# pkuyzy/ESC-GNN

Hardware: AMD Instinct MI355X
Metric: graphs/sec + edges-aggregated/sec, NestedGIN_eff h=3 bs=128 @1/2/4/8 GPU (higher is better)
Workload: dtype f32; 1 GPU; count_cycle-shaped random regular graphs (n in 10/15/20/30), target=triangles, NestedGIN_eff h=3 layers=4 hidden=256, bs=128 per GPU (configs[1]); global_batch=128, parallelism=dp1 graph-sharded, rccl_ranks=1, ranks=1

## Files before the change

esc-gnn_amd/csrc/common.h:

```cpp
#pragma once
#include <hip/hip_runtime.h>
#include <hip/hip_ext.h>
#include <stdint.h>
#include <stdio.h>
#include <stdarg.h>

#include "../../include/escgnn_hip.h"

namespace esc {

constexpr int WAVE = 64;

#ifndef ESC_NODE_PRIO
#define ESC_NODE_PRIO 2
#endif
#define ESC_PRIO() __builtin_amdgcn_s_setprio(ESC_NODE_PRIO)

void set_error(const char* fmt, ...);

#define ESC_REQUIRE(cond, ...)                    \
  do {                                            \
    if (!(cond)) {                                \
      esc::set_error(__VA_ARGS__);                \
      return ESC_EINVAL;                          \
// ... 5 lines not shown
    hipError_t err__ = hipGetLastError();                                   \
    if (err__ != hipSuccess) {                                              \
      esc::set_error("%s: launch failed: %s", name, hipGetErrorString(err__)); \
      return ESC_ELAUNCH;                                                   \
    }                                                                       \
  } while (0)

inline bool aligned16(const void* p) { return (reinterpret_cast<uintptr_t>(p) & 15) == 0; }
inline int64_t cdiv(int64_t a, int64_t b) { return (a + b - 1) / b; }

bool prof_slot(int kind, hipEvent_t* start, hipEvent_t* stop);
unsigned long long* prof_span_next(int kind);
#define ESC_SPAN_WGS 2048
#define ESC_SPAN_WAVES 8192
#define ESC_SPAN_STRIDE (ESC_SPAN_WGS + ESC_SPAN_WAVES)
bool trace_launch();

void arm_launch_event(hipEvent_t ev);
hipEvent_t take_launch_event();

template <typename... KArgs, typename... Args>
inline void launch(int kind, void (*kernel)(KArgs...), dim3 grid, dim3 block, size_t lds, hipStream_t s,
                   Args... args) {
  hipEvent_t a = nullptr, b = nullptr;
  hipEvent_t done = take_launch_event();
  if (done != nullptr) {
    hipStreamCaptureStatus cap = hipStreamCaptureStatusNone;
    if (hipStreamIsCapturing(s, &cap) != hipSuccess || cap != hipStreamCaptureStatusNone) { arm_launch_event(done); done = nullptr; }
  }
  if (prof_slot(kind, &a, &b)) {
    hipExtLaunchKernelGGL(kernel, grid, block, (unsigned)lds, s, a, b, 0, static_cast<KArgs>(args)...);
    if (done != nullptr) (void)hipEventRecord(done, s);
  } else if (done != nullptr) {
    hipExtLaunchKernelGGL(kernel, grid, block, (unsigned)lds, s, nullptr, done, 0, static_cast<KArgs>(args)...);
  } else {
    hipLaunchKernelGGL(kernel, grid, block, (unsigned)lds, s, static_cast<KArgs>(args)...);
  }
  if (trace_launch()) {
    const char* name = hipKernelNameRefByPtr(reinterpret_cast<const void*>(kernel), s);
    fprintf(stderr, "[esc] %s grid (%u,%u,%u) block %u lds %zu stream %p ...", name ? name : "?", grid.x, grid.y, grid.z, block.x, lds, (void*)s);
    fflush(stderr);
    const hipError_t e = hipStreamSynchronize(s);
    fprintf(stderr, " %s\n", e == hipSuccess ? "done" : hipGetErrorString(e));
  }
}

struct BnCounters {
  int n = 0;
  int64_t* p[ESC_MAX_BN_COUNTERS] = {};
};
int bag_bwd_classify_counted(const int32_t* c_row, int64_t Z, int64_t H, int64_t rows, float* partials, const BnCounters& cnt,
                             void* stream);

__device__ __forceinline__ int lane_id() { return threadIdx.x & 63; }

__device__ __forceinline__ int uniform(int v) { return __builtin_amdgcn_readfirstlane(v); }

__device__ __forceinline__ float wave_sum(float v) {
#pragma unroll
  for (int o = 32; o > 0; o >>= 1) v += __shfl_xor(v, o, 64);
  return v;
}
__device__ __forceinline__ double wave_sum(double v) {
#pragma unroll
  for (int o = 32; o > 0; o >>= 1) v += __shfl_xor(v, o, 64);
  return v;
}

unsigned* tickets(int n);
int gemm_lds_floor();
void set_gemm_lds_floor(int bytes);
int edge_lds_floor();
int node_lds_floor();
void set_node_lds_floor(int bytes);
void set_edge_lds_floor(int bytes);
int norm_rowblock_cap();
void set_norm_rowblock_cap(int v);
bool bn_bwd_one_launch();
void set_bn_bwd_one_launch(int on);
bool bn_bwd_fold();
void set_bn_bwd_fold(int on);
bool last_block_finalize();
void set_last_block_finalize(int on);
void set_linear_knob(int knob, int value);

__device__ __forceinline__ void store_agent(float2* p, float2 v) {
  const unsigned long long bits = ((unsigned long long)__float_as_uint(v.y) << 32) | __float_as_uint(v.x);
  __hip_atomic_store(reinterpret_cast<unsigned long long*>(p), bits, __ATOMIC_RELAXED, __HIP_MEMORY_SCOPE_AGENT);
}

__device__ __forceinline__ bool grid_last_block(unsigned* counter, unsigned nblocks) {
  __shared__ unsigned s_ticket;
  __builtin_amdgcn_s_waitcnt(0x0F70);
  __syncthreads();
  if (threadIdx.x == 0) s_ticket = __hip_atomic_fetch_add(counter, 1u, __ATOMIC_RELAXED, __HIP_MEMORY_SCOPE_AGENT);
  __syncthreads();
  const bool last = s_ticket == nblocks - 1;
  if (last) {
    __builtin_amdgcn_fence(__ATOMIC_ACQUIRE, "agent");
    if (threadIdx.x == 0) *counter = 0;
  }
  return last;
}

__device__ __forceinline__ void chan_merge(double& n, double& mu, double& m2, double nb, double mub, double m2b) {
  if (nb == 0.0) return;
  const double tot = n + nb;
  const double delta = mub - mu;
  mu += delta * nb / tot;
  m2 += m2b + delta * delta * n * nb / tot;
  n = tot;
}


struct BnFoldDev {
  const float2* partials;
  int P, block_rows, M, C;
  float eps, momentum;
  const float* gamma; const float* beta;
  float* mean; float* invstd; float* scale; float* shift; float* running_mean; float* running_var;
};
__device__ __forceinline__ void bn_fold_column(const BnFoldDev& f, int col, bool writer, float& sc, float& sh) {
  const int full = f.M / f.block_rows;
  double n = 0.0, mu = 0.0, m2 = 0.0;
  if (full > 0) {
    const double pivot = (double)f.partials[col].x;
    double S1 = 0.0, S2 = 0.0, SM = 0.0;
    constexpr int CH = 40;
    for (int p0 = 0; p0 < full; p0 += CH) {
      float2 v[CH];
#pragma unroll
      for (int u = 0; u < CH; ++u) v[u] = f.partials[(size_t)min(p0 + u, full - 1) * f.C + col];
#pragma unroll
      for (int u = 0; u < CH; ++u) {
        if (p0 + u < full) { const double d = (double)v[u].x - pivot; S1 += d; S2 += d * d; SM += (double)v[u].y; }
      }
    }
    n = (double)f.block_rows * full;
    mu = pivot + S1 / full;
    m2 = SM + (double)f.block_rows * (S2 - S1 * S1 / full);
    if (m2 < 0.0) m2 = 0.0;
  }
  if (f.M > f.block_rows * full) {
    const float2 v = f.partials[(size_t)full * f.C + col];
    chan_merge(n, mu, m2, (double)(f.M - f.block_rows * full), (double)v.x, (double)v.y);
  }
  const float is = (float)(1.0 / sqrt(m2 / (double)f.M + (double)f.eps));
  sc = (f.gamma ? f.gamma[col] : 1.f) * is;
  sh = (f.beta ? f.beta[col] : 0.f) - (float)mu * sc;
  if (writer) {
    f.mean[col] = (float)mu;
    f.invstd[col] = is;
    if (f.scale) { f.scale[col] = sc; f.shift[col] = sh; }
    if (f.running_mean) f.running_mean[col] = (1.f - f.momentum) * f.running_mean[col] + f.momentum * (float)mu;
    if (f.running_var) f.running_var[col] = (1.f - f.momentum) * f.running_var[col] + f.momentum * (float)(m2 / (double)(f.M - 1));
  }
}

struct BnbDev {
  const float* x; int ldx;
  const float* mean; const float* invstd; const float* scale; const float* shift;
  const float2* coef;
  int relu;
};
struct BnStatDev {
  float2* partial;
// ... 20 lines not shown
```

esc-gnn_amd/csrc/linear_mfma.hip:

```cpp
#include "common.h"
#include <cstdlib>
#include "linear_plan.h"
#include "gemm_tile.h"
#include "gemm_dma.h"
#include "linear_small.h"
#include "linear_narrow.h"

namespace esc {

using plan::Flags;
using plan::Op;
using plan::Plan;

static plan::PlanKnobs g_plan;
void set_linear_knob(int knob, int value) {
  if (knob == 11) g_plan.use_dma = value;
  else g_plan.knob[knob] = value;
}
static const plan::PlanKnobs& knobs() {
  static const bool env_read = [] {
    if (getenv("ESC_BIG_MIN_WGS")) g_plan.big_min_wgs = atoll(getenv("ESC_BIG_MIN_WGS"));
    if (getenv("ESC_TILE160")) g_plan.tile160 = atoi(getenv("ESC_TILE160"));
    if (getenv("ESC_TILE160_MIN_WGS")) g_plan.tile160_min_wgs = atoll(getenv("ESC_TILE160_MIN_WGS"));
    return true;
// ... 69 lines not shown
static void dma_fill_dx(dma::GArgs& g, const float* dY, int64_t ld_dy, const float* W, int64_t ld_w, int64_t M, int64_t N,
                        int64_t K, float* dX, int64_t ld_dx, int accumulate) {
  g.A = dY; g.lda = (int)ld_dy; g.B = W; g.ldb = (int)ld_w; g.C = dX; g.ldc = (int)ld_dx;
  g.M = (int)M; g.N = (int)K; g.R = (int)N; g.red_per_split = (int)N; g.accumulate = accumulate;
}
static void dma_fill_dw(dma::GArgs& g, const float* dY, int64_t ld_dy, const float* X, int64_t ld_x, const float* in_scale,
                        const float* in_shift, int64_t M, int64_t N, int64_t K, float* slabs, const Plan& p) {
  g.A = dY; g.lda = (int)ld_dy; g.B = X; g.ldb = (int)ld_x; g.C = slabs; g.ldc = (int)K;
  g.pro_scale = in_scale; g.pro_shift = in_shift; g.db_part = slabs + (size_t)p.splits * N * K;
  g.M = (int)N; g.N = (int)K; g.R = (int)M; g.red_per_split = p.per_split; g.accumulate = 0;
}

enum NarrowForm { NARROW_PLAIN, NARROW_FOLD, NARROW_L1 };
static void launch_narrow_fwd(NarrowForm form, const float* X, int64_t ld_x, const float* W, int64_t ld_w, const float* bias,
                              const float* in_scale, const float* in_shift, int64_t M, int64_t N, int64_t K, float* Y, int64_t ld_y,
                              const BnFoldDev& fold, const NarrowL1& l1, hipStream_t s) {
  const unsigned blocks = (unsigned)(cdiv(M, 16) < 2048 ? cdiv(M, 16) : 2048);
#define ESC_NARROW_FWD(...) \
  esc::launch(ESC_K_LINEAR, linear_narrow_fwd<__VA_ARGS__>, dim3(blocks), dim3(256), 0, s, X, ld_x, W, ld_w, bias, in_scale, in_shift, (int)M, (int)N, (int)K, Y, ld_y, fold, l1)
  if (form == NARROW_L1) ESC_NARROW_FWD(1, true, false, true);
  else if (form == NARROW_FOLD) { if (N == 1) ESC_NARROW_FWD(1, true, true); else ESC_NARROW_FWD(4, true, true); }
  else if (N == 1) { if (in_scale) ESC_NARROW_FWD(1, true); else ESC_NARROW_FWD(1, false); }
  else { if (in_scale) ESC_NARROW_FWD(4, true); else ESC_NARROW_FWD(4, false); }
#undef ESC_NARROW_FWD
}

static hipError_t launch_dma_fwd(const Plan& p, const dma::GArgs& g, hipStream_t s) {
  const bool pro = g.pro_scale != nullptr;
#define ESC_DMA_FWD(PRO, ...) dma::launch_gemm<__VA_ARGS__, false, false, PRO, true, false>(g, 0, s)
#define ESC_DMA_FWD_FROM(PRO, ...) dma::launch_gemm<__VA_ARGS__, false, false, PRO, true, false, true>(g, 0, s)
  const bool big = p.family == plan::F_DMA128;
  if (g.c_init != nullptr) {
    if (big) return pro ? ESC_DMA_FWD_FROM(1, ESC_T128) : ESC_DMA_FWD_FROM(0, ESC_T128);
    return pro ? ESC_DMA_FWD_FROM(1, ESC_T64) : ESC_DMA_FWD_FROM(0, ESC_T64);
  }
  if (g.fold.partials != nullptr) return big ? ESC_DMA_FWD(3, ESC_T128) : ESC_DMA_FWD(3, ESC_T64);
  switch (p.family) {
    case plan::F_DMA64X32:
      return pro ? dma::launch_gemm<ESC_T64X32, false, false, 1, false, false>(g, 0, s)
                 : dma::launch_gemm<ESC_T64X32, false, false, 0, false, false>(g, 0, s);
    case plan::F_DMA160: return pro ? ESC_DMA_FWD(1, ESC_T160) : ESC_DMA_FWD(0, ESC_T160);
    case plan::F_DMA128: return pro ? ESC_DMA_FWD(1, ESC_T128) : ESC_DMA_FWD(0, ESC_T128);
    case plan::F_DMA128X64: return ESC_DMA_FWD(0, ESC_T128X64);
    default: return pro ? ESC_DMA_FWD(1, ESC_T64) : ESC_DMA_FWD(0, ESC_T64);
  }
#undef ESC_DMA_FWD
#undef ESC_DMA_FWD_FROM
}
static dma::GArgs dma_fwd_args(const float* X, int64_t ld_x, const float* W, int64_t ld_w, const float* bias, const float* in_scale,
                               const float* in_shift, int64_t M, int64_t N, int64_t K, float* Y, int64_t ld_y, float* col_stats) {
  dma::GArgs g{};
  g.A = X; g.lda = (int)ld_x; g.B = W; g.ldb = (int)ld_w; g.C = Y; g.ldc = (int)ld_y; g.bias = bias;
  g.pro_scale = in_scale; g.pro_shift = in_shift; g.col_stats = reinterpret_cast<float2*>(col_stats);
  g.M = (int)M; g.N = (int)N; g.R = (int)K; g.red_per_split = (int)K; g.accumulate = 0;
  return g;
}

static int launch_smalln_dx(const float* dY, int64_t ld_dy, const float* W, int64_t ld_w, int64_t M, int64_t N, int64_t K, float* dX,
                            int64_t ld_dx, int accumulate, const BnbDev& bd, int act, const char* what, hipStream_t s) {
  const size_t lds = (size_t)(32 + small::SMALL_MAX) * (N + 4) * sizeof(float);
  static size_t raised[3] = {64 * 1024, 64 * 1024, 64 * 1024};
  hipError_t e = hipSuccess;
  if (act == 0) e = dma::raise_lds(small::smalln_dx<small::SMALL_MAX>, lds, raised[0]);
  if (act != 0) e = dma::raise_lds(small::smalln_dx<small::SMALL_MAX, 1>, lds, raised[1]);
  if (e == hipSuccess && act == 2) e = dma::raise_lds(small::smalln_dx<small::SMALL_MAX, 2>, lds, raised[2]);
  if (dma_check(e, what) != hipSuccess) return ESC_ELAUNCH;
  auto kern = act == 0 ? small::smalln_dx<small::SMALL_MAX> : (act == 2 ? small::smalln_dx<small::SMALL_MAX, 2> : small::smalln_dx<small::SMALL_MAX, 1>);
  esc::launch(ESC_K_LINEAR, kern, dim3((unsigned)cdiv(M, 32)), dim3(256), lds, s, dY, ld_dy, W, ld_w, (int)M, (int)N, (int)K, dX, ld_dx, accumulate, bd);
  return ESC_OK;
}

static void launch_wgrad_small(const float* dY, int64_t ld_dy, const float* X, int64_t ld_x, const float* in_scale, const float* in_shift,
                               int64_t M, int64_t N, int64_t K, float* slabs, const Plan& p, const BnbDev& bd, int act, hipStream_t s) {
  float* db_part = slabs + (size_t)p.splits * N * K;
  const bool small_k = K <= small::SMALL_MAX;
  const dim3 grid((unsigned)p.splits, (unsigned)cdiv(small_k ? N : K, 256));
#define ESC_WGRAD_SMALL(...) \
  esc::launch(ESC_K_LINEAR, small::wgrad_small<small::SMALL_MAX, __VA_ARGS__>, grid, dim3(256), 0, s, dY, ld_dy, X, ld_x, in_scale, in_shift, (int)M, (int)N, (int)K, slabs, db_part, bd)
  if (act == 2)      { if (in_scale) ESC_WGRAD_SMALL(true, true, 2); else ESC_WGRAD_SMALL(true, false, 2); }
  else if (act == 1) { if (in_scale) ESC_WGRAD_SMALL(true, true, 1); else ESC_WGRAD_SMALL(true, false, 1); }
  else if (small_k)  { if (in_scale) ESC_WGRAD_SMALL(true, true); else ESC_WGRAD_SMALL(true, false); }
  else               { if (in_scale) ESC_WGRAD_SMALL(false, true); else ESC_WGRAD_SMALL(false, false); }
#undef ESC_WGRAD_SMALL
}

static int reduce_slabs(const Plan& p, const float* slabs, int64_t N, int64_t K, float* dW, int64_t ld_dw, float* db, esc_reduce_job* defer,
                        void* stream) {
  esc_reduce_job now;
  esc_reduce_job* j = defer ? defer : &now;
  j->slabs = slabs; j->n = N * K; j->splits = p.splits; j->cols = K; j->dw = dW; j->ld_dw = ld_dw;
  j->db_part = slabs + (size_t)p.splits * N * K; j->rows = N; j->db = db;
  return defer ? ESC_OK : esc_slab_reduce_jobs(j, 1, stream);
}

}

using namespace esc;

extern "C" {

int esc_debug_gemm_occupancy(int tile_id) {
  int n = -1;
#define ESC_OCC(I)                                                                                                              \
  {                                                                                                                             \
    constexpr plan::Tile t = plan::R01_TILE[I];                                                                                 \
    auto kern = gemm_tile_kernel<t.bm, t.bn, t.wm, t.wn, t.bk, true, true, false, false>;                                       \
    const size_t lds = 2 * (KContigTile<t.bm, t.bk>::FLOATS + KContigTile<t.bn, t.bk>::FLOATS) * sizeof(float);                 \
    if (lds > 64 * 1024) (void)hipFuncSetAttribute((const void*)kern, hipFuncAttributeMaxDynamicSharedMemorySize, (int)lds);    \
    (void)hipOccupancyMaxActiveBlocksPerMultiprocessor(&n, kern, 256, lds);                                                     \
  }
  switch (tile_id) {
    case 0: ESC_OCC(0) break;
    case 2: ESC_OCC(2) break;
    case 3: ESC_OCC(3) break;
    case 4: ESC_OCC(4) break;
    default: ESC_OCC(1) break;
  }
#undef ESC_OCC
  return n;
}

static int linear_fwd_impl(const float* X, int64_t ld_x, const float* W, int64_t ld_w, const float* bias,
                           const float* in_scale, const float* in_shift, int64_t M, int64_t N, int64_t K,
                           float* Y, int64_t ld_y, float* col_stats, const esc_bn_fuse* bn, void* stream) {
  ESC_REQUIRE(X && W && Y, "esc_linear_fwd: null pointer");
  ESC_REQUIRE(M >= 0 && N > 0 && K > 0 && ld_x >= K && ld_w >= K && ld_y >= N, "esc_linear_fwd: bad sizes M=%ld N=%ld K=%ld", (long)M, (long)N, (long)K);
  ESC_REQUIRE((in_scale == nullptr) == (in_shift == nullptr), "esc_linear_fwd: in_scale/in_shift must come together");
  ESC_REQUIRE(col_stats == nullptr || N > 32, "esc_linear_fwd: col_stats needs N > 32");
  ESC_REQUIRE(M < (1LL << 31) && N < (1LL << 31) && K < (1LL << 31), "esc_linear_fwd: dimension too large");
  ESC_REQUIRE(bn == nullptr || (col_stats && bn->mean && bn->invstd && M > 1), "esc_linear_bn_fwd: needs col_stats, mean, invstd and M > 1");
  ESC_REQUIRE(bn == nullptr || ((bn->scale == nullptr) == (bn->shift == nullptr)), "esc_linear_bn_fwd: scale/shift must come together");
  if (M == 0) return ESC_OK;
  hipStream_t s = (hipStream_t)stream;
  Flags f = pro_flags(in_scale, in_shift);
  f.col_stats = col_stats != nullptr; f.bn = bn != nullptr; f.last_block_finalize = last_block_finalize();
  const Plan p = plan::plan_fwd(knobs(), Op{X, ld_x}, Op{W, ld_w}, M, N, K, f);
  switch (p.family) {
    case plan::F_NARROW:
      launch_narrow_fwd(NARROW_PLAIN, X, ld_x, W, ld_w, bias, in_scale, in_shift, M, N, K, Y, ld_y, BnFoldDev{}, NarrowL1{}, s);
      ESC_CHECK_LAUNCH("esc_linear_fwd.narrow");
      break;
    case plan::F_SMALLK:
      esc::launch(ESC_K_LINEAR, small::smallk_fwd<small::SMALL_MAX>, dim3((unsigned)cdiv(M, small::ROWS_FWD), (unsigned)cdiv(N, 256)),
                  dim3(256), 0, s, X, ld_x, W, ld_w, bias, (int)M, (int)N, (int)K, Y, ld_y, reinterpret_cast<float2*>(col_stats));
      ESC_CHECK_LAUNCH("esc_linear_fwd.smallk");
      break;
    case plan::F_DMA64X32: case plan::F_DMA64: case plan::F_DMA128: case plan::F_DMA128X64: case plan::F_DMA160:
      if (dma_check(launch_dma_fwd(p, dma_fwd_args(X, ld_x, W, ld_w, bias, in_scale, in_shift, M, N, K, Y, ld_y, col_stats), s), "esc_linear_fwd") != hipSuccess)
        return ESC_ELAUNCH;
      break;
    default: {
      GemmArgs g{};
      g.A = X; g.lda = ld_x; g.B = W; g.ldb = ld_w; g.C = Y; g.ldc = ld_y; g.bias = bias;
      g.pro_scale = in_scale; g.pro_shift = in_shift; g.db_part = nullptr;
      g.col_stats = p.family == plan::F_R01_ROWSTATS ? nullptr : reinterpret_cast<float2*>(col_stats);
      g.rowsC = (int)M; g.colsC = (int)N; g.red = (int)K; g.red_per_split = (int)K; g.accumulate = 0;
      g.a_vec = plan::vec_ok(Op{X, ld_x}) && f.pro_aligned;
      g.b_vec = plan::vec_ok(Op{W, ld_w}); g.c_slab = 0;
      if (p.family == plan::F_R01_BN) {
        g.fin.tickets = tickets((int)cdiv(N, p.bn));
        ESC_REQUIRE(g.fin.tickets != nullptr, "esc_linear_bn_fwd: no ticket counters");
        g.fin.row_tiles = (int)cdiv(M, p.bm);
        g.fin.eps = bn->eps; g.fin.momentum = bn->momentum; g.fin.mean = bn->mean; g.fin.invstd = bn->invstd;
        g.fin.running_mean = bn->running_mean; g.fin.running_var = bn->running_var; g.fin.gamma = bn->gamma;
        g.fin.beta = bn->beta; g.fin.scale = bn->scale; g.fin.shift = bn->shift;
      }
// ... 221 lines not shown
      dma_fill_dw(a.dw, dY, ld_dy, X, ld_x, in_scale, in_shift, M, N, K, slabs, p);
      hipError_t e;
      if (p.family == plan::F_DMA160_DUAL)      e = in_scale ? dma::launch_dual<ESC_T160, true>(a, 0, s) : dma::launch_dual<ESC_T160, false>(a, 0, s);
      else if (p.family == plan::F_DMA128_DUAL) e = in_scale ? dma::launch_dual<ESC_T128, true>(a, 0, s) : dma::launch_dual<ESC_T128, false>(a, 0, s);
      else                                      e = in_scale ? dma::launch_dual<ESC_T64, true>(a, 0, s) : dma::launch_dual<ESC_T64, false>(a, 0, s);
      if (dma_check(e, "esc_linear_bwd_both") != hipSuccess) return ESC_ELAUNCH;
      break;
    }
    case plan::F_SPLIT: {
      const int rc = weight_impl(dY, ld_dy, X, ld_x, in_scale, in_shift, M, N, K, dW, ld_dw, db, slabs, defer, stream);
      if (rc || dX == nullptr) return rc;
      return esc_linear_bwd_input(dY, ld_dy, W, ld_w, M, N, K, dX, ld_dx, accumulate, stream);
    }
    default: {
      ESC_REQUIRE(M > 0 && ld_dy >= N && ld_x >= K && ld_w >= K && ld_dx >= K && ld_dw >= K, "esc_linear_bwd_both: bad sizes");
      ESC_REQUIRE((in_scale == nullptr) == (in_shift == nullptr), "esc_linear_bwd_both: in_scale/in_shift must come together");
      ESC_REQUIRE(M < (1LL << 31) && N < (1LL << 31) && K < (1LL << 31), "esc_linear_bwd_both: dimension too large");
      DualArgs a{};
      a.dx = r01_dx_args(dY, ld_dy, W, ld_w, M, N, K, dX, ld_dx, accumulate);
      a.dw = r01_dw_args(dY, ld_dy, X, ld_x, in_scale, in_shift, M, N, K, slabs, p);
      a.dx_nx = (int)cdiv(K, p.bn); a.dx_ny = (int)cdiv(M, p.bm);
      a.dw_nx = (int)cdiv(K, p.bn); a.dw_ny = (int)cdiv(N, p.bm); a.dw_nz = p.splits;
#define ESC_DUAL(I, PRO) launch_dual<plan::R01_TILE[I].bm, plan::R01_TILE[I].bn, plan::R01_TILE[I].wm, plan::R01_TILE[I].wn, plan::R01_TILE[I].bk, PRO>(a, s)
      if (p.tile == 5)      { if (in_scale) ESC_DUAL(5, true); else ESC_DUAL(5, false); }
      else if (p.tile == 1) { if (in_scale) ESC_DUAL(1, true); else ESC_DUAL(1, false); }
      else                  { if (in_scale) ESC_DUAL(4, true); else ESC_DUAL(4, false); }
#undef ESC_DUAL
      ESC_CHECK_LAUNCH("esc_linear_bwd_both.tiles");
    }
  }
  return reduce_slabs(p, slabs, N, K, dW, ld_dw, db, defer, stream);
}

int esc_linear_bwd_both(const float* dY, int64_t ld_dy, const float* X, int64_t ld_x, const float* in_scale,
                        const float* in_shift, const float* W, int64_t ld_w, int64_t M, int64_t N, int64_t K,
                        float* dX, int64_t ld_dx, int accumulate, float* dW, int64_t ld_dw, float* db,
                        float* slabs, void* stream) {
  return both_impl(dY, ld_dy, X, ld_x, in_scale, in_shift, W, ld_w, M, N, K, dX, ld_dx, accumulate, dW, ld_dw, db, slabs,
                   nullptr, stream);
}

int esc_linear_bwd_both_deferred(const float* dY, int64_t ld_dy, const float* X, int64_t ld_x, const float* in_scale,
                                 const float* in_shift, const float* W, int64_t ld_w, int64_t M, int64_t N, int64_t K,
                                 float* dX, int64_t ld_dx, int accumulate, float* dW, int64_t ld_dw, float* db,
                                 float* slabs, esc_reduce_job* job, void* stream) {
  ESC_REQUIRE(job, "esc_linear_bwd_both_deferred: null job");
  return both_impl(dY, ld_dy, X, ld_x, in_scale, in_shift, W, ld_w, M, N, K, dX, ld_dx, accumulate, dW, ld_dw, db, slabs,
                   job, stream);
}

static Plan plan_both_bn(const float* dOut, int64_t ld_dout, const esc_bn_bwd_fused* b, const float* X, int64_t ld_x, const float* W,
                         int64_t ld_w, int64_t M, int64_t N, int64_t K, const float* dX, int64_t ld_dx, const float* slabs,
                         const esc_bn_bwd_next* n) {
  plan::BnOps bo{};
  plan::NextOps no{};
  if (b) bo = plan::BnOps{b->x, b->ld_x, b->mean, b->invstd, b->scale, b->shift, b->coef, b->relu};
  if (n) no = plan::NextOps{n->partial, n->x, n->ld_x, n->mean, n->invstd, n->scale, n->shift, n->relu};
  return plan::plan_both_bn(knobs(), Op{dOut, ld_dout}, b ? &bo : nullptr, Op{X, ld_x}, Op{W, ld_w}, Op{dX, ld_dx}, slabs, n ? &no : nullptr,
                            M, N, K);
}

int esc_linear_bwd_both_bn_ok(const float* dOut, int64_t ld_dout, const esc_bn_bwd_fused* bn, const float* X, int64_t ld_x,
                              const float* W, int64_t ld_w, int64_t M, int64_t N, int64_t K, const float* dX, int64_t ld_dx,
                              const float* slabs, const esc_bn_bwd_next* next) {
  return plan_both_bn(dOut, ld_dout, bn, X, ld_x, W, ld_w, M, N, K, dX, ld_dx, slabs, next).ok ? 1 : 0;
}

int64_t esc_linear_bwd_bn_block_rows(int64_t M, int64_t N, int64_t K) { return plan::bwd_bn_block_rows(M, N, K); }

int esc_linear_bwd_both_bn(const float* dOut, int64_t ld_dout, const esc_bn_bwd_fused* bn, const float* X, int64_t ld_x,
                           const float* in_scale, const float* in_shift, const float* W, int64_t ld_w, int64_t M,
                           int64_t N, int64_t K, float* dX, int64_t ld_dx, int accumulate, float* dW, int64_t ld_dw,
                           float* db, float* slabs, esc_reduce_job* defer, const esc_bn_bwd_next* next, void* stream) {
  ESC_REQUIRE(dOut && X && W && dW && slabs, "esc_linear_bwd_both_bn: null pointer");
  ESC_REQUIRE((in_scale == nullptr) == (in_shift == nullptr), "esc_linear_bwd_both_bn: in_scale/in_shift must come together");
  ESC_REQUIRE(ld_dw >= K, "esc_linear_bwd_both_bn: bad sizes");
  const Plan p = plan_both_bn(dOut, ld_dout, bn, X, ld_x, W, ld_w, M, N, K, dX, ld_dx, slabs, next);
  ESC_REQUIRE(p.ok, "esc_linear_bwd_both_bn: shape / alignment not served (M=%ld N=%ld K=%ld) - use esc_bn_bwd + esc_linear_bwd_both", (long)M, (long)N, (long)K);
  hipStream_t s = (hipStream_t)stream;
  const BnbDev bd = bn ? BnbDev{bn->x, (int)bn->ld_x, bn->mean, bn->invstd, bn->scale, bn->shift, reinterpret_cast<const float2*>(bn->coef), bn->relu}
                       : BnbDev{};
  if (p.family == plan::F_SMALL_BN) {
    const int act = bd.relu == 2 ? 2 : 1;
    launch_wgrad_small(dOut, ld_dout, X, ld_x, in_scale, in_shift, M, N, K, slabs, p, bd, act, s);
    ESC_CHECK_LAUNCH("esc_linear_bwd_both_bn.small");
    if (dX != nullptr) {
      ESC_TRY_(launch_smalln_dx(dOut, ld_dout, W, ld_w, M, N, K, dX, ld_dx, accumulate, bd, act, "esc_linear_bwd_both_bn", s));
      ESC_CHECK_LAUNCH("esc_linear_bwd_both_bn.smalln");
    }
    return reduce_slabs(p, slabs, N, K, dW, ld_dw, db, defer, stream);
  }
  dma::DualArgs a{};
  dma_fill_dx(a.dx, dOut, ld_dout, W, ld_w, M, N, K, dX, ld_dx, accumulate);
  dma_fill_dw(a.dw, dOut, ld_dout, X, ld_x, in_scale, in_shift, M, N, K, slabs, p);
  a.dx.bnb = bd; a.dw.bnb = bd;
  if (next)
    a.dx.bst = BnStatDev{reinterpret_cast<float2*>(next->partial), next->x, (int)next->ld_x, next->mean, next->invstd, next->scale, next->shift, next->relu};
  hipError_t e;
#define ESC_T64_2STAGE 64, 64, 32, 2, 2, 2, 2
  if (p.family == plan::F_DMA128_BN) {
    if (next) e = in_scale ? dma::launch_dual<ESC_T128, true, true, true>(a, 0, s) : dma::launch_dual<ESC_T128, false, true, true>(a, 0, s);
    else      e = in_scale ? dma::launch_dual<ESC_T128, true, true, false>(a, 0, s) : dma::launch_dual<ESC_T128, false, true, false>(a, 0, s);
  } else {
    if (bn == nullptr) e = in_scale ? dma::launch_dual<ESC_T64, true, false, true>(a, 0, s) : dma::launch_dual<ESC_T64, false, false, true>(a, 0, s);
    else if (next)     e = in_scale ? dma::launch_dual<ESC_T64_2STAGE, true, true, true>(a, 0, s) : dma::launch_dual<ESC_T64_2STAGE, false, true, true>(a, 0, s);
    else               e = in_scale ? dma::launch_dual<ESC_T64_2STAGE, true, true, false>(a, 0, s) : dma::launch_dual<ESC_T64_2STAGE, false, true, false>(a, 0, s);
  }
#undef ESC_T64_2STAGE
  if (dma_check(e, "esc_linear_bwd_both_bn") != hipSuccess) return ESC_ELAUNCH;
  return reduce_slabs(p, slabs, N, K, dW, ld_dw, db, defer, stream);
}

}
```

esc-gnn_amd/csrc/linear_small.h:

```cpp
#pragma once
#include "common.h"
#include "linear_plan.h"

namespace esc {
namespace small {


template <int KMAX>
__global__ __launch_bounds__(256) void smallk_fwd(const float* __restrict__ X, int64_t ldx, const float* __restrict__ W,
                                                  int64_t ldw, const float* __restrict__ bias, int M, int N, int K,
                                                  float* __restrict__ Y, int64_t ldy, float2* __restrict__ col_stats) {
  ESC_PRIO();
  __shared__ float xs[ROWS_FWD * KMAX];
  const int n = blockIdx.y * 256 + threadIdx.x;
  const int r0 = blockIdx.x * ROWS_FWD;
  const int rows = min(ROWS_FWD, M - r0);
  for (int i = threadIdx.x; i < ROWS_FWD * KMAX; i += 256) {
    const int r = i / KMAX, k = i % KMAX;
    xs[i] = (r < rows && k < K) ? X[(size_t)(r0 + r) * ldx + k] : 0.f;
  }
  float w[KMAX];
#pragma unroll
  for (int k = 0; k < KMAX; ++k) w[k] = (n < N && k < K) ? W[(size_t)n * ldw + k] : 0.f;
  const float b = (bias != nullptr && n < N) ? bias[n] : 0.f;
// ... 55 lines not shown
    float b_mu = 0.f, b_a = 0.f, b_ms = 0.f, b_mh = 1.f, b_k1 = 0.f, b_k2 = 0.f;
    if constexpr (BNB != 0) {
      const float2 kk = bnb.coef[t];
      b_mu = bnb.mean[t]; b_a = bnb.scale[t]; b_k1 = kk.x; b_k2 = bnb.invstd[t] * kk.y;
      if (bnb.relu) { b_ms = b_a; b_mh = bnb.shift[t]; }
    }
#pragma unroll 4
    for (int r = 0; r < rows; ++r) {
      float v = V[(size_t)(r0 + r) * ldv + t];
      if constexpr (BNB == 1) v = bnb_apply(v, bnb.x[(size_t)(r0 + r) * bnb.ldx + t], b_mu, b_a, b_ms, b_mh, b_k1, b_k2);
      if constexpr (BNB == 2) v = bnb_apply_elu(v, bnb.x[(size_t)(r0 + r) * bnb.ldx + t], b_mu, b_a, b_ms, b_mh, b_k1, b_k2);
      if constexpr (PRO && !SMALL_K) v = fmaxf(fmaf(v, psc, psh), 0.f);
      if constexpr (SMALL_K) colsum += v;
#pragma unroll
      for (int q = 0; q < SMAX; ++q) acc[q] = fmaf(us[r * SMAX + q], v, acc[q]);
    }
    float* out = slabs + (size_t)split * N * K;
#pragma unroll
    for (int q = 0; q < SMAX; ++q)
      if (q < S) out[SMALL_K ? (size_t)t * K + q : (size_t)q * K + t] = acc[q];
    if constexpr (SMALL_K) db_part[(size_t)split * N + t] = colsum;
  }
  if constexpr (!SMALL_K) {
    if (blockIdx.y == 0 && (int)threadIdx.x < N) {
      float s = 0.f;
      for (int r = 0; r < rows; ++r) s += us[r * SMAX + threadIdx.x];
      db_part[(size_t)split * N + threadIdx.x] = s;
    }
  }
}

template <int KMAX, int BNB = 0>
__global__ __launch_bounds__(256) void smalln_dx(const float* __restrict__ dY, int64_t lddy, const float* __restrict__ W,
                                                 int64_t ldw, int M, int N, int K, float* __restrict__ dX, int64_t lddx,
                                                 int accumulate, BnbDev bnb) {
  ESC_PRIO();
  extern __shared__ __attribute__((aligned(16))) float sm[];
  const int ldn = N + 4;
  float* ys = sm;
  float* wt = sm + 32 * ldn;
  const int r0 = blockIdx.x * 32;
  const int rows = min(32, M - r0);
  for (int i = threadIdx.x; i < rows * (N / 4); i += 256) {
    const int r = i / (N / 4), c = (i % (N / 4)) * 4;
    float4 v = *reinterpret_cast<const float4*>(dY + (size_t)(r0 + r) * lddy + c);
    if constexpr (BNB != 0) {
      const float4 x = *reinterpret_cast<const float4*>(bnb.x + (size_t)(r0 + r) * bnb.ldx + c);
      const float4 mu = *reinterpret_cast<const float4*>(bnb.mean + c), a = *reinterpret_cast<const float4*>(bnb.scale + c);
      const float4 is = *reinterpret_cast<const float4*>(bnb.invstd + c);
      const float4 k01 = *reinterpret_cast<const float4*>(bnb.coef + c), k23 = *reinterpret_cast<const float4*>(bnb.coef + c + 2);
      float4 ms = make_float4(0.f, 0.f, 0.f, 0.f), mh = make_float4(1.f, 1.f, 1.f, 1.f);
      if (bnb.relu) { ms = a; mh = *reinterpret_cast<const float4*>(bnb.shift + c); }
      if constexpr (BNB == 2) {
        v.x = bnb_apply_elu(v.x, x.x, mu.x, a.x, ms.x, mh.x, k01.x, is.x * k01.y); v.y = bnb_apply_elu(v.y, x.y, mu.y, a.y, ms.y, mh.y, k01.z, is.y * k01.w);
        v.z = bnb_apply_elu(v.z, x.z, mu.z, a.z, ms.z, mh.z, k23.x, is.z * k23.y); v.w = bnb_apply_elu(v.w, x.w, mu.w, a.w, ms.w, mh.w, k23.z, is.w * k23.w);
      } else {
        v.x = bnb_apply(v.x, x.x, mu.x, a.x, ms.x, mh.x, k01.x, is.x * k01.y); v.y = bnb_apply(v.y, x.y, mu.y, a.y, ms.y, mh.y, k01.z, is.y * k01.w);
        v.z = bnb_apply(v.z, x.z, mu.z, a.z, ms.z, mh.z, k23.x, is.z * k23.y); v.w = bnb_apply(v.w, x.w, mu.w, a.w, ms.w, mh.w, k23.z, is.w * k23.w);
      }
    }
    *reinterpret_cast<float4*>(ys + r * ldn + c) = v;
  }
  for (int i = threadIdx.x; i < N * K; i += 256) wt[(i % K) * ldn + (i / K)] = W[(size_t)(i / K) * ldw + (i % K)];
  __syncthreads();
  const int r = threadIdx.x >> 3, ks = threadIdx.x & 7;
  if (r >= rows) return;
#pragma unroll
  for (int kk = 0; kk < KMAX / 8; ++kk) {
    const int k = ks + kk * 8;
    if (k >= K) break;
    float a0 = 0.f, a1 = 0.f, a2 = 0.f, a3 = 0.f;
    for (int c = 0; c < N; c += 4) {
      const float4 y = *reinterpret_cast<const float4*>(ys + r * ldn + c);
      const float4 w = *reinterpret_cast<const float4*>(wt + k * ldn + c);
      a0 = fmaf(y.x, w.x, a0); a1 = fmaf(y.y, w.y, a1); a2 = fmaf(y.z, w.z, a2); a3 = fmaf(y.w, w.w, a3);
    }
    float v = (a0 + a1) + (a2 + a3);
    float* dst = dX + (size_t)(r0 + r) * lddx + k;
    if (accumulate) v += *dst;
    *dst = v;
  }
}

}
}
```

esc-gnn_amd/csrc/runtime.hip:

```cpp
#include "common.h"
#include "linear_plan.h"
#include <algorithm>
#include <cstdlib>

#include <mutex>
#include <vector>

namespace esc {

static thread_local char g_err[512] = "";

void set_error(const char* fmt, ...) {
  va_list ap;
  va_start(ap, fmt);
  vsnprintf(g_err, sizeof(g_err), fmt, ap);
  va_end(ap);
}

struct ProfState {
  bool on = false;
  std::vector<hipEvent_t> start, stop;
  size_t used = 0;
};
static ProfState g_prof[ESC_K_COUNT];
static std::mutex g_prof_mu;

bool prof_slot(int k, hipEvent_t* start, hipEvent_t* stop) {
  if (k == ESC_K_GEMM_EDGE && !g_prof[k].on) k = ESC_K_LINEAR;
  if (k < 0 || k >= ESC_K_COUNT || !g_prof[k].on) return false;
  std::lock_guard<std::mutex> lk(g_prof_mu);
  ProfState& p = g_prof[k];
  if (p.used == p.start.size()) {
    hipEvent_t a, b;
    if (hipEventCreate(&a) != hipSuccess || hipEventCreate(&b) != hipSuccess) return false;
    p.start.push_back(a);
    p.stop.push_back(b);
  }
  *start = p.start[p.used];
  *stop = p.stop[p.used];
  ++p.used;
  return true;
}

struct SpanState { unsigned long long* dev = nullptr; size_t cap = 0; };
static SpanState g_span[ESC_K_COUNT];
unsigned long long* prof_span_next(int k) {
  if (k < 0 || k >= ESC_K_COUNT) return nullptr;
  std::lock_guard<std::mutex> lk(g_prof_mu);
  if (!g_prof[k].on || g_span[k].dev == nullptr || g_prof[k].used >= g_span[k].cap) return nullptr;
  return g_span[k].dev + g_prof[k].used * ESC_SPAN_STRIDE;
}
__global__ void span_init_kernel(unsigned long long* p, size_t n) {
  const size_t i = (size_t)blockIdx.x * blockDim.x + threadIdx.x;
  if (i < n) p[i] = (i % ESC_SPAN_STRIDE) < ESC_SPAN_WGS ? ~0ULL : 0ULL;
}

constexpr int TICKET_POOL = 4096;
static unsigned* g_tickets[64] = {};
static int g_ticket_pos[64] = {};
static std::mutex g_ticket_mu;

static int g_last_block = 0;
bool last_block_finalize() { return g_last_block != 0; }
void set_last_block_finalize(int on) { g_last_block = on != 0; }

static thread_local int g_gemm_lds_floor = 0;
int gemm_lds_floor() { return g_gemm_lds_floor; }
void set_gemm_lds_floor(int bytes) { g_gemm_lds_floor = bytes < 0 ? 0 : (bytes > 160 * 1024 ? 160 * 1024 : bytes); }
static int g_edge_lds_floor = 52 * 1024;
int edge_lds_floor() { return g_edge_lds_floor; }
static thread_local int g_node_lds_floor = 0;
int node_lds_floor() { return g_node_lds_floor; }
void set_node_lds_floor(int bytes) { g_node_lds_floor = bytes < 0 ? 0 : (bytes > 160 * 1024 ? 160 * 1024 : bytes); }
void set_edge_lds_floor(int bytes) { g_edge_lds_floor = bytes < 0 ? 0 : bytes; }

static thread_local hipEvent_t g_launch_event = nullptr;
void arm_launch_event(hipEvent_t ev) { g_launch_event = ev; }
hipEvent_t take_launch_event() { hipEvent_t ev = g_launch_event; g_launch_event = nullptr; return ev; }

static const bool g_trace_launch = getenv("ESC_TRACE_LAUNCH") != nullptr && atoi(getenv("ESC_TRACE_LAUNCH")) != 0;
bool trace_launch() { return g_trace_launch; }
static int g_bn_bwd_one = getenv("ESC_BN_BWD_ONE") ? atoi(getenv("ESC_BN_BWD_ONE")) : 0;
bool bn_bwd_one_launch() { return g_bn_bwd_one != 0; }
void set_bn_bwd_one_launch(int on) { g_bn_bwd_one = on != 0; }
static int g_bn_bwd_fold = 0;
bool bn_bwd_fold() { return g_bn_bwd_fold != 0; }
void set_bn_bwd_fold(int on) { g_bn_bwd_fold = on != 0; }
static int g_norm_rowblock_cap = 256;
int norm_rowblock_cap() { return g_norm_rowblock_cap; }
void set_norm_rowblock_cap(int v) { g_norm_rowblock_cap = v < 1 ? 1 : (v > 512 ? 512 : v); }

unsigned* tickets(int n) {
  int dev = 0;
  if (hipGetDevice(&dev) != hipSuccess || dev < 0 || dev >= 64 || n <= 0 || n > TICKET_POOL) return nullptr;
  std::lock_guard<std::mutex> lk(g_ticket_mu);
  if (g_tickets[dev] == nullptr) {
    unsigned* p = nullptr;
    if (hipMalloc(&p, sizeof(unsigned) * TICKET_POOL) != hipSuccess) return nullptr;
    if (hipMemset(p, 0, sizeof(unsigned) * TICKET_POOL) != hipSuccess) { (void)hipFree(p); return nullptr; }
    g_tickets[dev] = p;
  }
  if (g_ticket_pos[dev] + n > TICKET_POOL) g_ticket_pos[dev] = 0;
  unsigned* out = g_tickets[dev] + g_ticket_pos[dev];
  g_ticket_pos[dev] += n;
  return out;
}

}

extern "C" {

int esc_tune_set(int knob, int value) {
  if (knob == 8) { esc::set_last_block_finalize(value); return ESC_OK; }
  if (knob == 9) { esc::set_norm_rowblock_cap(value); return ESC_OK; }
  if (knob == 12) { esc::set_bn_bwd_fold(value); return ESC_OK; }
  if (knob == 13) { esc::set_bn_bwd_one_launch(value); return ESC_OK; }
  if (knob == 10) { esc::set_edge_lds_floor(value); return ESC_OK; }
  ESC_REQUIRE(knob == 11 || (knob >= 0 && knob < esc::plan::KNOB_COUNT), "esc_tune_set: unknown knob %d", knob);
  esc::set_linear_knob(knob, value);
  return ESC_OK;
}

int esc_abi_version(void) { return ESC_ABI_VERSION; }
const char* esc_last_error(void) { return esc::g_err; }

int esc_prof_enable(int kind, int on) {
  ESC_REQUIRE(kind >= 0 && kind < ESC_K_COUNT, "esc_prof_enable: bad kind %d", kind);
  std::lock_guard<std::mutex> lk(esc::g_prof_mu);
  esc::g_prof[kind].on = on != 0;
  return ESC_OK;
}

int esc_prof_reset(int kind) {
  ESC_REQUIRE(kind >= 0 && kind < ESC_K_COUNT, "esc_prof_reset: bad kind %d", kind);
  std::lock_guard<std::mutex> lk(esc::g_prof_mu);
  esc::g_prof[kind].used = 0;
  return ESC_OK;
}

int esc_prof_read(int kind, int64_t* launches, double* total_ms) {
  ESC_REQUIRE(kind >= 0 && kind < ESC_K_COUNT && launches && total_ms, "esc_prof_read: bad argument");
  std::lock_guard<std::mutex> lk(esc::g_prof_mu);
  esc::ProfState& p = esc::g_prof[kind];
  double tot = 0;
  for (size_t i = 0; i < p.used; ++i) {
    if (hipEventSynchronize(p.stop[i]) != hipSuccess) {
      esc::set_error("esc_prof_read: event sync failed");
      return ESC_ELAUNCH;
    }
    float ms = 0;
    (void)hipEventElapsedTime(&ms, p.start[i], p.stop[i]);
    tot += ms;
  }
  *launches = (int64_t)p.used;
  *total_ms = tot;
  return ESC_OK;
}

int esc_prof_span_arm(int kind, int64_t launches, void* stream) {
  ESC_REQUIRE(kind >= 0 && kind < ESC_K_COUNT && launches > 0 && launches <= 4096, "esc_prof_span_arm: 1..4096 launches");
  std::lock_guard<std::mutex> lk(esc::g_prof_mu);
  esc::SpanState& sp = esc::g_span[kind];
  if (sp.cap < (size_t)launches) {
    if (sp.dev) (void)hipFree(sp.dev);
    sp.dev = nullptr; sp.cap = 0;
    if (hipMalloc(&sp.dev, (size_t)launches * ESC_SPAN_STRIDE * sizeof(unsigned long long)) != hipSuccess) { esc::set_error("esc_prof_span_arm: allocation failed"); return ESC_ELAUNCH; }
    sp.cap = (size_t)launches;
  }
  const size_t n = sp.cap * ESC_SPAN_STRIDE;
  hipLaunchKernelGGL(esc::span_init_kernel, dim3((unsigned)((n + 255) / 256)), dim3(256), 0, (hipStream_t)stream, sp.dev, n);
  return ESC_OK;
}

int64_t esc_prof_span_read(int kind, double* us_out, int64_t cap) {
  if (kind < 0 || kind >= ESC_K_COUNT || us_out == nullptr || cap <= 0) return 0;
  std::lock_guard<std::mutex> lk(esc::g_prof_mu);
  esc::SpanState& sp = esc::g_span[kind];
  const size_t n = std::min<size_t>(std::min<size_t>(esc::g_prof[kind].used, sp.cap), (size_t)cap);
  if (n == 0 || sp.dev == nullptr) return 0;
  std::vector<unsigned long long> h(n * ESC_SPAN_STRIDE);
  if (hipMemcpy(h.data(), sp.dev, n * ESC_SPAN_STRIDE * sizeof(unsigned long long), hipMemcpyDeviceToHost) != hipSuccess) return 0;
  int dev = 0, khz = 100000;
  (void)hipGetDevice(&dev);
  if (hipDeviceGetAttribute(&khz, hipDeviceAttributeWallClockRate, dev) != hipSuccess || khz <= 0) khz = 100000;
  for (size_t i = 0; i < n; ++i) {
    unsigned long long lo = ~0ULL, hi = 0ULL;
    const unsigned long long* q = h.data() + i * ESC_SPAN_STRIDE;
    for (int w = 0; w < ESC_SPAN_WGS; ++w) lo = std::min(lo, q[w]);
    for (int w = 0; w < ESC_SPAN_WAVES; ++w) hi = std::max(hi, q[ESC_SPAN_WGS + w]);
    us_out[i] = (hi > lo && lo != ~0ULL) ? (double)(hi - lo) * 1e3 / (double)khz : 0.0;
  }
  return (int64_t)n;
}

int64_t esc_prof_read_all(int kind, double* ms_out, int64_t cap) {
  if (kind < 0 || kind >= ESC_K_COUNT || ms_out == nullptr || cap <= 0) return 0;
  std::lock_guard<std::mutex> lk(esc::g_prof_mu);
  esc::ProfState& p = esc::g_prof[kind];
  int64_t n = 0;
  for (size_t i = 0; i < p.used && n < cap; ++i) {
// ... 10 lines not shown
```

Measured before the change: 134,500 graphs/s.

## Fuse small-K BatchNorm backward weight-grad and input-grad into one kernel

After: 135,100 graphs/s (median of 6 runs). No clear change (+0.5%).

```diff
diff --git a/esc-gnn_amd/csrc/common.h b/esc-gnn_amd/csrc/common.h
--- a/esc-gnn_amd/csrc/common.h
+++ b/esc-gnn_amd/csrc/common.h
@@ -111,6 +111,8 @@
 void set_bn_bwd_fold(int on);
 bool last_block_finalize();
 void set_last_block_finalize(int on);
+bool small_bn_onepass();
+void set_small_bn_onepass(int on);
 void set_linear_knob(int knob, int value);
 
 __device__ __forceinline__ void store_agent(float2* p, float2 v) {
diff --git a/esc-gnn_amd/csrc/linear_mfma.hip b/esc-gnn_amd/csrc/linear_mfma.hip
--- a/esc-gnn_amd/csrc/linear_mfma.hip
+++ b/esc-gnn_amd/csrc/linear_mfma.hip
@@ -175,6 +175,33 @@
   else if (small_k)  { if (in_scale) ESC_WGRAD_SMALL(true, true); else ESC_WGRAD_SMALL(true, false); }
   else               { if (in_scale) ESC_WGRAD_SMALL(false, true); else ESC_WGRAD_SMALL(false, false); }
 #undef ESC_WGRAD_SMALL
+}
+
+constexpr size_t LDS_LIMIT = 160 * 1024;
+template <bool PRO, int BNB, bool DX>
+static hipError_t launch_bn_onepass_as(const float* dOut, int64_t ld_dout, const float* X, int64_t ld_x, const float* in_scale,
+                                       const float* in_shift, const float* W, int64_t ld_w, int64_t M, int64_t N, int64_t K, float* dX,
+                                       int64_t ld_dx, int accumulate, float* slabs, const Plan& p, const BnbDev& bd, hipStream_t s) {
+  static size_t raised = 64 * 1024;
+  const size_t lds = small::onepass_lds_bytes(N);
+  const hipError_t e = dma::raise_lds(small::bn_onepass<PRO, BNB, DX>, lds, raised);
+  if (e != hipSuccess) return e;
+  esc::launch(ESC_K_LINEAR, small::bn_onepass<PRO, BNB, DX>, dim3((unsigned)p.splits), dim3(small::ONEPASS_THREADS), lds, s, dOut, ld_dout, X,
+              ld_x, in_scale, in_shift, W, ld_w, (int)M, (int)N, (int)K, dX, ld_dx, accumulate, slabs, slabs + (size_t)p.splits * N * K, bd);
+  return hipSuccess;
+}
+static hipError_t launch_bn_onepass(const float* dOut, int64_t ld_dout, const float* X, int64_t ld_x, const float* in_scale,
+                                    const float* in_shift, const float* W, int64_t ld_w, int64_t M, int64_t N, int64_t K, float* dX,
+                                    int64_t ld_dx, int accumulate, float* slabs, const Plan& p, const BnbDev& bd, int act, hipStream_t s) {
+#define ESC_ONEPASS(...) launch_bn_onepass_as<__VA_ARGS__>(dOut, ld_dout, X, ld_x, in_scale, in_shift, W, ld_w, M, N, K, dX, ld_dx, accumulate, slabs, p, bd, s)
+  const bool pro = in_scale != nullptr;
+  if (dX != nullptr) {
+    if (act == 2) return pro ? ESC_ONEPASS(true, 2, true) : ESC_ONEPASS(false, 2, true);
+    return pro ? ESC_ONEPASS(true, 1, true) : ESC_ONEPASS(false, 1, true);
+  }
+  if (act == 2) return pro ? ESC_ONEPASS(true, 2, false) : ESC_ONEPASS(false, 2, false);
+  return pro ? ESC_ONEPASS(true, 1, false) : ESC_ONEPASS(false, 1, false);
+#undef ESC_ONEPASS
 }
 
 static int reduce_slabs(const Plan& p, const float* slabs, int64_t N, int64_t K, float* dW, int64_t ld_dw, float* db, esc_reduce_job* defer,
@@ -562,6 +589,13 @@
                        : BnbDev{};
   if (p.family == plan::F_SMALL_BN) {
     const int act = bd.relu == 2 ? 2 : 1;
+    if (small_bn_onepass() && small::onepass_lds_bytes(N) <= LDS_LIMIT) {
+      if (dma_check(launch_bn_onepass(dOut, ld_dout, X, ld_x, in_scale, in_shift, W, ld_w, M, N, K, dX, ld_dx, accumulate, slabs, p, bd, act, s),
+                    "esc_linear_bwd_both_bn") != hipSuccess)
+        return ESC_ELAUNCH;
+      ESC_CHECK_LAUNCH("esc_linear_bwd_both_bn.onepass");
+      return reduce_slabs(p, slabs, N, K, dW, ld_dw, db, defer, stream);
+    }
     launch_wgrad_small(dOut, ld_dout, X, ld_x, in_scale, in_shift, M, N, K, slabs, p, bd, act, s);
     ESC_CHECK_LAUNCH("esc_linear_bwd_both_bn.small");
     if (dX != nullptr) {
diff --git a/esc-gnn_amd/csrc/linear_small.h b/esc-gnn_amd/csrc/linear_small.h
--- a/esc-gnn_amd/csrc/linear_small.h
+++ b/esc-gnn_amd/csrc/linear_small.h
@@ -161,5 +161,128 @@
   }
 }
 
-}
-}
+constexpr int ONEPASS_THREADS = 512;
+constexpr int ONEPASS_BATCH = 4;
+inline size_t onepass_lds_bytes(int64_t N) { return (size_t)((32 + SMALL_MAX + 1) * (N + 4) + ROWS_WGRAD * SMALL_MAX) * sizeof(float); }
+
+template <bool PRO, int BNB, bool DX>
+__global__ __launch_bounds__(ONEPASS_THREADS) __attribute__((amdgpu_waves_per_eu(2, 4)))
+void bn_onepass(const float* __restrict__ dY, int64_t lddy, const float* __restrict__ X, int64_t ldx, const float* __restrict__ sc,
+                const float* __restrict__ sh, const float* __restrict__ W, int64_t ldw, int M, int N, int K, float* __restrict__ dX,
+                int64_t lddx, int accumulate, float* __restrict__ slabs, float* __restrict__ db_part, BnbDev bnb) {
+  static_assert(BNB == 1 || BNB == 2, "the one-pass kernel serves the fused BatchNorm backward only");
+  static_assert(ROWS_WGRAD == 32 && SMALL_MAX == 16, "slab height and k-slots of the two kernels this one replaces");
+  ESC_PRIO();
+  extern __shared__ __attribute__((aligned(16))) float sm[];
+  const int ldn = N + 4;
+  float* ts = sm;
+  float* wt = sm + 32 * ldn;
+  float* av = sm + (32 + SMALL_MAX) * ldn;
+  float* xs = av + ldn;
+  const int tid = threadIdx.x;
+  const int split = blockIdx.x;
+  const int r0 = split * ROWS_WGRAD;
+  const int rows = min(ROWS_WGRAD, M - r0);
+  float xv = 0.f;
+  const int xr = tid / SMALL_MAX, xk = tid % SMALL_MAX;
+  if (xr < rows && xk < K) xv = X[(size_t)(r0 + xr) * ldx + xk];
+  const int nq = N / 4;
+  const int lanes = ONEPASS_THREADS / nq;
+  const int cq = tid % nq, rl = tid / nq;
+  if (rl < lanes && rl < rows) {
+    const int c = cq * 4;
+    float4 g[ONEPASS_BATCH], x[ONEPASS_BATCH];
+    auto load_batch = [&](int rb) {
+#pragma unroll
+      for (int j = 0; j < ONEPASS_BATCH; ++j) {
+        const int r = min(rb + j * lanes, rows - 1);
+        g[j] = *reinterpret_cast<const float4*>(dY + (size_t)(r0 + r) * lddy + c);
+        x[j] = *reinterpret_cast<const float4*>(bnb.x + (size_t)(r0 + r) * bnb.ldx + c);
+      }
+    };
+    load_batch(rl);
+    const float4 mu = *reinterpret_cast<const float4*>(bnb.mean + c), a = *reinterpret_cast<const float4*>(bnb.scale + c);
+    const float4 is = *reinterpret_cast<const float4*>(bnb.invstd + c);
+    const float4 k01 = *reinterpret_cast<const float4*>(bnb.coef + c), k23 = *reinterpret_cast<const float4*>(bnb.coef + c + 2);
+    float4 ms = make_float4(0.f, 0.f, 0.f, 0.f), mh = make_float4(1.f, 1.f, 1.f, 1.f);
+    if (bnb.relu) { ms = a; mh = *reinterpret_cast<const float4*>(bnb.shift + c); }
+    const float k2x = is.x * k01.y, k2y = is.y * k01.w, k2z = is.z * k23.y, k2w = is.w * k23.w;
+    if (rl == 0) *reinterpret_cast<float4*>(av + c) = a;
+    for (int rb = rl;;) {
+#pragma unroll
+      for (int j = 0; j < ONEPASS_BATCH; ++j) {
+        const int r = min(rb + j * lanes, rows - 1);
+        float4 v = g[j];
+        if constexpr (BNB == 2) {
+          v.x = bnb_apply_elu(v.x, x[j].x, mu.x, 1.f, ms.x, mh.x, k01.x, k2x); v.y = bnb_apply_elu(v.y, x[j].y, mu.y, 1.f, ms.y, mh.y, k01.z, k2y);
+          v.z = bnb_apply_elu(v.z, x[j].z, mu.z, 1.f, ms.z, mh.z, k23.x, k2z); v.w = bnb_apply_elu(v.w, x[j].w, mu.w, 1.f, ms.w, mh.w, k23.z, k2w);
+        } else {
+          v.x = bnb_apply(v.x, x[j].x, mu.x, 1.f, ms.x, mh.x, k01.x, k2x); v.y = bnb_apply(v.y, x[j].y, mu.y, 1.f, ms.y, mh.y, k01.z, k2y);
+          v.z = bnb_apply(v.z, x[j].z, mu.z, 1.f, ms.z, mh.z, k23.x, k2z); v.w = bnb_apply(v.w, x[j].w, mu.w, 1.f, ms.w, mh.w, k23.z, k2w);
+        }
+        *reinterpret_cast<float4*>(ts + r * ldn + c) = v;
+      }
+      rb += lanes * ONEPASS_BATCH;
+      if (rb >= rows) break;
+      load_batch(rb);
+    }
+  }
+  if constexpr (DX)
+    for (int i = tid; i < N * K; i += ONEPASS_THREADS) wt[(i % K) * ldn + (i / K)] = W[(size_t)(i / K) * ldw + (i % K)];
+  if constexpr (PRO)
+    if (xr < rows && xk < K) xv = fmaxf(fmaf(xv, sc[xk], sh[xk]), 0.f);
+  xs[tid] = xv;
+  __syncthreads();
+  if (tid < 256) {
+    float* out = slabs + (size_t)split * N * K;
+    for (int n = tid; n < N; n += 256) {
+      const float a = av[n];
+      float acc[SMALL_MAX];
+#pragma unroll
+      for (int q = 0; q < SMALL_MAX; ++q) acc[q] = 0.f;
+      float colsum = 0.f;
+#pragma unroll 4
+      for (int r = 0; r < rows; ++r) {
+        const float t = ts[r * ldn + n];
+        const float v = __fmul_rn(a, t);
+        colsum = fmaf(a, t, colsum);
+#pragma unroll
+        for (int q = 0; q < SMALL_MAX; ++q) acc[q] = fmaf(xs[r * SMALL_MAX + q], v, acc[q]);
+      }
+#pragma unroll
+      for (int q = 0; q < SMALL_MAX; ++q)
+        if (q < K) out[(size_t)n * K + q] = acc[q];
+      db_part[(size_t)split * N + n] = colsum;
+    }
+  } else if constexpr (DX) {
+    const int u = tid - 256;
+    const int r = u >> 3, k0 = u & 7;
+    if (r >= rows || k0 >= K) return;
+    const bool two = k0 + 8 < K;
+    const float* tr = ts + r * ldn;
+    const float* w0 = wt + k0 * ldn;
+    const float* w1 = wt + (two ? k0 + 8 : k0) * ldn;
+    float a0 = 0.f, a1 = 0.f, a2 = 0.f, a3 = 0.f, b0 = 0.f, b1 = 0.f, b2 = 0.f, b3 = 0.f;
+    for (int c = 0; c < N; c += 4) {
+      const float4 t = *reinterpret_cast<const float4*>(tr + c);
+      const float4 a = *reinterpret_cast<const float4*>(av + c);
+      const float4 p = *reinterpret_cast<const float4*>(w0 + c);
+      const float4 q = *reinterpret_cast<const float4*>(w1 + c);
+      const float yx = __fmul_rn(a.x, t.x), yy = __fmul_rn(a.y, t.y), yz = __fmul_rn(a.z, t.z), yw = __fmul_rn(a.w, t.w);
+      a0 = fmaf(yx, p.x, a0); a1 = fmaf(yy, p.y, a1); a2 = fmaf(yz, p.z, a2); a3 = fmaf(yw, p.w, a3);
+      b0 = fmaf(yx, q.x, b0); b1 = fmaf(yy, q.y, b1); b2 = fmaf(yz, q.z, b2); b3 = fmaf(yw, q.w, b3);
+    }
+    float* dst = dX + (size_t)(r0 + r) * lddx + k0;
+    float v = (a0 + a1) + (a2 + a3);
+    if (accumulate) v += *dst;
+    *dst = v;
+    if (two) {
+      float v1 = (b0 + b1) + (b2 + b3);
+      if (accumulate) v1 += dst[8];
+      dst[8] = v1;
+    }
+  }
+}
+
+}
+}
diff --git a/esc-gnn_amd/csrc/runtime.hip b/esc-gnn_amd/csrc/runtime.hip
--- a/esc-gnn_amd/csrc/runtime.hip
+++ b/esc-gnn_amd/csrc/runtime.hip
@@ -86,6 +86,9 @@
 static int g_bn_bwd_fold = 0;
 bool bn_bwd_fold() { return g_bn_bwd_fold != 0; }
 void set_bn_bwd_fold(int on) { g_bn_bwd_fold = on != 0; }
+static int g_small_bn_onepass = 1;
+bool small_bn_onepass() { return g_small_bn_onepass != 0; }
+void set_small_bn_onepass(int on) { g_small_bn_onepass = on != 0; }
 static int g_norm_rowblock_cap = 256;
 int norm_rowblock_cap() { return g_norm_rowblock_cap; }
 void set_norm_rowblock_cap(int v) { g_norm_rowblock_cap = v < 1 ? 1 : (v > 512 ? 512 : v); }
@@ -116,6 +119,7 @@
   if (knob == 12) { esc::set_bn_bwd_fold(value); return ESC_OK; }
   if (knob == 13) { esc::set_bn_bwd_one_launch(value); return ESC_OK; }
   if (knob == 10) { esc::set_edge_lds_floor(value); return ESC_OK; }
+  if (knob == 14) { esc::set_small_bn_onepass(value); return ESC_OK; }
   ESC_REQUIRE(knob == 11 || (knob >= 0 && knob < esc::plan::KNOB_COUNT), "esc_tune_set: unknown knob %d", knob);
   esc::set_linear_knob(knob, value);
   return ESC_OK;
```
